# LauraFJulia/TFT_vs_Fund

Measured on AMD Instinct MI355X. Metric: triplet-hypotheses/sec (linearTFT+R,t) at N=200 corresp., higher is better.
Workload: dtype f64; 1 GPU; configs[1]: batch of 10000 synthetic triplets x 200 correspondences, sigma=1px, linearTFT + R_t_from_TFT (LinearTFTPoseEstimation without Reconst), one batch per GPU; batch_per_gpu=10000, correspondences=200, streams=2 (consecutive batches alternate between streams and may overlap), gather=none (1 GPU), failed_triplets=0, warmup_steps_run=2560

## Files before the change

tft_vs_fund_amd/csrc/f_rows_kernel.h:

```cpp
#pragma once
#include "tft_rows_kernel.h"
#include "tft_rows_exact_kernel.h"
#include "f_kernel.h"

namespace tff {

__device__ __forceinline__ void rows_distances_moments_f(const RowSrc& s, const int N, const double (&c)[6], double* nrm, double* nrm2, double* mom) {
    const int p = rows_p();
    double acc[80];
#pragma unroll
    for (int k = 0; k < 80; ++k) acc[k] = 0.0;
    double d[3] = {0.0, 0.0, 0.0};
    Pt6 pnext = rows_load(s, (p < N) ? p : 0);
#pragma unroll 1
    for (int i = p; i < N; i += ROWL) {
        const Pt6 q = pnext;
        if (i + ROWL < N) pnext = rows_load(s, i + ROWL);
        const double x1 = q.v[0] - c[0], y1 = q.v[1] - c[1];
        const double x2 = q.v[2] - c[2], y2 = q.v[3] - c[3];
        const double x3 = q.v[4] - c[4], y3 = q.v[5] - c[5];
        const double m1[6] = {x1 * x1, x1 * y1, x1, y1 * y1, y1, 1.0};
        const double m2[6] = {x2 * x2, x2 * y2, x2, y2 * y2, y2, 1.0};
        const double m3[6] = {x3 * x3, x3 * y3, x3, y3 * y3, y3, 1.0};
        d[0] += sqrt_nonneg(m1[0] + m1[3]); d[1] += sqrt_nonneg(m2[0] + m2[3]); d[2] += sqrt_nonneg(m3[0] + m3[3]);
// ... 67 lines not shown
        const int v2 = p + 1;
        Mat3 F;
#pragma unroll
        for (int r = 0; r < 3; ++r)
#pragma unroll
            for (int c = 0; c < 3; ++c) F.m[r][c] = Fm[9 * p + 3 * r + c];
        F = mat3_mul(mat3_mul(mat3_T(normal_matrix(nrm2, v2)), F), normal_matrix(nrm2, 0));
        double v3[3], fv[3];
        nok = null3<false>(F, v3);
#pragma unroll
        for (int r = 0; r < 3; ++r) fv[r] = F.m[r][0] * v3[0] + F.m[r][1] * v3[1] + F.m[r][2] * v3[2];
#pragma unroll
        for (int r = 0; r < 3; ++r)
#pragma unroll
            for (int c = 0; c < 3; ++c) F.m[r][c] -= fv[r] * v3[c];
        if constexpr (X_FRAME) {
            double nn = 0.0;
#pragma unroll
            for (int r = 0; r < 3; ++r)
#pragma unroll
                for (int c = 0; c < 3; ++c) nn += F.m[r][c] * F.m[r][c];
            const double sc = rsqrt(nn);
#pragma unroll
            for (int r = 0; r < 3; ++r)
#pragma unroll
                for (int c = 0; c < 3; ++c) Fm[9 * p + 3 * r + c] = F.m[r][c] * sc;
        } else {
            F = mat3_mul(mat3_mul(mat3_T(normal_matrix(w->nrm, v2)), F), normal_matrix(w->nrm, 0));
            const Mat3 E = mat3_mul(mat3_mul(mat3_T(load_K(w->calm, v2)), F), load_K(w->calm, 0));
#pragma unroll
            for (int r = 0; r < 3; ++r)
#pragma unroll
                for (int c = 0; c < 3; ++c) rt->Ein[9 * p + 3 * r + c] = E.m[r][c];
        }
    }
    const bool bad = row_any(!nok);
    wave_sync();
    return ok && !bad;
}

template <bool RAGGED>
__device__ __forceinline__ void linear_f_pose_rows(const LinearTftArgs& a) {
    TFF_DYNAMIC_LDS(double, smem);
    if (a.retry_zero && blockIdx.x == 0 && threadIdx.x == 0) *a.retry_zero = 0;
    const int p = lane_id() & 15, row = lane_id() >> 4;
    RowLds* w = reinterpret_cast<RowLds*>(smem) + row;
    RowRt* rt = reinterpret_cast<RowRt*>(w->ov);
    for (long blk = blockIdx.x; RAGGED ? rows_ragged_slot(a, blk) < a.rrange[1] : blk * ROW_TRIPLETS < a.B; blk += gridDim.x) {
        const int N = RAGGED ? rows_ragged_n(a, blk) : opaque_int(a.N);
        const RowJob j = RAGGED ? rows_begin_ragged(a, w, blk) : rows_begin(a, w, blk, N);
        int status;
        if (N < 8) {
            status = ST_TOO_FEW;
            rows_store_nan<RAGGED>(a, j, N);
        } else {
            {
                double cen[6];
                rows_centroids(j.src, N, cen);
                rows_distances_moments_f(j.src, N, cen, w->nrm, w->pa, w->mom);
            }
            wave_sync();
            bool ok = rows_linear_f_middle(w, rt, w->t, w->pa, j.dbg);
            rows_recover_prepare(w, rt);
            status = rows_pose_tail<true, false, RAGGED>(a, w, rt, j, N, ok);
        }
        if (p == 0 && j.valid) {
            if (a.iter) a.iter[j.b] = 0;
            a.status[j.b] = status;
            if (status == ST_RETRY && a.retry_list) a.retry_list[atomicAdd(a.retry_count, 1)] = (int)j.b;
        }
    }
}
__global__ void __launch_bounds__(64, 2) k_linear_f_pose_rows(const LinearTftArgs a) { linear_f_pose_rows<false>(a); }
__global__ void __launch_bounds__(64, 2) k_linear_f_pose_rows_ragged(const LinearTftArgs a) { linear_f_pose_rows<true>(a); }

template <int M>
__device__ __forceinline__ void rows_f_system_chunk(const RowSrc& s, const int N, const int base, const double* nrm, const double* nrm2, const int p, const int ca,
                                                    const int cb, const int pair, double* Rp, double* xch) {
    double a0[M], a1[M];
#pragma unroll
    for (int r = 0; r < M; ++r) {
        const int i = base + r;
        const Pt6 q = premap(premap(rows_load(s, (i < N) ? i : 0), nrm), nrm2);
        const double h1 = (ca == 0) ? q.v[0] : (ca == 1) ? q.v[1] : 1.0;
        const double h2 = (cb == 0) ? (pair ? q.v[4] : q.v[2]) : (cb == 1) ? (pair ? q.v[5] : q.v[3]) : 1.0;
        a0[r] = (i < N && p < 9) ? h1 * h2 : 0.0;
        a1[r] = 0.0;
    }
    rows_qr_append<9, M>(a0, a1, Rp, xch);
}

__device__ __forceinline__ bool rows_linear_f_middle_exact(RowLds* w, RowRt* rt, const RowSrc& s, const int N, double* Fm, double* nrm2, double* dbg) {
    const int p = opaque_lane_int(rows_p());
    double* Rp = w->ov;
    double* xch = w->mom;
    double* dinv = w->mom + 32;
    {
        double sm[6] = {0, 0, 0, 0, 0, 0};
#pragma unroll 1
        for (int i = p; i < N; i += ROWL) {
            const Pt6 q = premap(rows_load(s, i), w->nrm);
#pragma unroll
            for (int k = 0; k < 6; ++k) sm[k] += q.v[k];
        }
        double c[6];
#pragma unroll
        for (int k = 0; k < 6; ++k) c[k] = row_sum16(sm[k]) / (double)N;
        double d[3] = {0.0, 0.0, 0.0};
#pragma unroll 1
        for (int i = p; i < N; i += ROWL) {
            const Pt6 q = premap(rows_load(s, i), w->nrm);
#pragma unroll
            for (int v = 0; v < 3; ++v) {
                const double dx = q.v[2 * v] - c[2 * v], dy = q.v[2 * v + 1] - c[2 * v + 1];
                d[v] += sqrt(dx * dx + dy * dy);
            }
        }
        const double r2c = sqrt(2.0);
#pragma unroll
        for (int v = 0; v < 3; ++v) {
            const double norm0 = row_sum16(d[v]) / (double)N;
            if (p == 3 * v) nrm2[3 * v] = r2c / norm0;
// ... 94 lines not shown
```

tft_vs_fund_amd/csrc/pose_common.h:

```cpp
#pragma once
#include "wave.h"
#include "small_la.h"
#include "wave_eig.h"
#include "row_eig.h"
#include "wave_qr.h"

namespace tff {

constexpr int FLAG_RECONST = 1;
constexpr int FLAG_JACOBI = 2;
constexpr int FLAG_STAGE_LDS = 4;
constexpr int FLAG_ONLY_RETRY = 8;
constexpr int FLAG_DBG_FP_HANDOVER = 64;
constexpr int FLAG_DBG_ADAPTIVE = 32;
constexpr int FLAG_XI_IN_LDS = 128;
constexpr int FLAG_GH_EXACT = 16;

constexpr int ST_OK = 0;
constexpr int ST_TOO_FEW = 1;
constexpr int ST_NONFINITE = 2;
constexpr int ST_NO_POSE = 3;
constexpr int ST_RETRY = 100;

constexpr int DBG_STRIDE = 128;
// ... 419 lines not shown
        double S[4][3];
#pragma unroll
        for (int r = 0; r < 4; ++r)
#pragma unroll
            for (int c = 0; c < 3; ++c) {
                if (c > r) continue;
                double v = b0[r] * b0[c] + b1[r] * b1[c];
                if (r < 3) v += a0[r] * a0[c] + a1[r] * a1[c];
                S[r][c] = v;
            }
        const double S33 = b0[3] * b0[3] + b1[3] * b1[3];
        const double tr3 = S[0][0] + S[1][1] + S[2][2];
        const double delta = 1e-14 * (tr3 + S33), pfloor = 1e-3 * delta + 1e-300;
        double L[4][3], inv[3];
#pragma unroll
        for (int j = 0; j < 3; ++j) {
            double d = S[j][j] + delta;
#pragma unroll
            for (int k = 0; k < j; ++k) d -= L[j][k] * L[j][k];
            d = fmax(d, pfloor);
            inv[j] = rsqrt_pos(d);
#pragma unroll
            for (int r = j + 1; r < 4; ++r) {
                double sv = S[r][j];
#pragma unroll
                for (int k = 0; k < j; ++k) sv -= L[r][k] * L[j][k];
                L[r][j] = sv * inv[j];
            }
        }
        double z[3];
#pragma unroll
        for (int r = 2; r >= 0; --r) {
            double sum = -L[3][r];
#pragma unroll
            for (int k = r + 1; k < 3; ++k) sum -= L[k][r] * z[k];
            z[r] = sum * inv[r];
        }
        const double d1 = z[2], d2 = R3[0] * z[0] + R3[1] * z[1] + R3[2] * z[2] + R3[3];
        const double d4 = S33 + delta - (L[3][0] * L[3][0] + L[3][1] * L[3][1] + L[3][2] * L[3][2]);
        const double zz = z[0] * z[0] + z[1] * z[1] + z[2] * z[2];
        const double idet = (inv[0] * inv[1]) * (inv[0] * inv[1]) * (inv[2] * inv[2]);
        const double trs = tr3 + 3.0 * delta;
        const double e = trs * trs * idet;
        const double Gp = 4.0 * (1.0 + zz) - d4 * e;
        const double rhs = 2.0 * d4 * e + 2.5e-14 * trs * e * Gp;
        const double dmin2 = fmin(d1 * d1, d2 * d2);
        const bool certain = Gp > 0.0 && dmin2 * Gp * Gp > rhs * rhs * zz;
        all_certain = all_certain && certain;
        score += (int)sgn(d1) + (int)sgn(d2);
    }
    return 2 * wave_sum_i(score) + (wave_any(!all_certain) ? 1 : 0);
}
struct VoteCam { double PB[12], R3[4]; };
struct VoteFactor { double L[4][3], inv[3], d4, z[3], pfloor; };
template <bool KEEP = false, bool CERT = true>
__device__ __forceinline__ void vote_one(const double (&SA)[6], const VoteCam& cam, const double x2, const double y2, int& score, bool& all_certain,
                                         VoteFactor* keep = nullptr) {
    double b0[4], b1[4];
#pragma unroll
    for (int c = 0; c < 4; ++c) { b0[c] = y2 * cam.PB[8 + c] - cam.PB[4 + c]; b1[c] = cam.PB[c] - x2 * cam.PB[8 + c]; }
    double S[4][3];
#pragma unroll
    for (int r = 0; r < 4; ++r)
#pragma unroll
        for (int c = 0; c < 3; ++c) {
            if (c > r) continue;
            double v = b0[r] * b0[c] + b1[r] * b1[c];
            if (r < 3) v += SA[r * (r + 1) / 2 + c];
            S[r][c] = v;
        }
    const double S33 = b0[3] * b0[3] + b1[3] * b1[3];
    const double tr3 = S[0][0] + S[1][1] + S[2][2];
    const double delta = 1e-14 * (tr3 + S33), pfloor = 1e-3 * delta + 1e-300;
    double L[4][3], inv[3];
#pragma unroll
    for (int j = 0; j < 3; ++j) {
        double d = S[j][j] + delta;
#pragma unroll
        for (int k = 0; k < j; ++k) d -= L[j][k] * L[j][k];
        d = fmax(d, pfloor);
        inv[j] = rsqrt_pos(d);
#pragma unroll
        for (int r = j + 1; r < 4; ++r) {
            double sv = S[r][j];
#pragma unroll
            for (int k = 0; k < j; ++k) sv -= L[r][k] * L[j][k];
            L[r][j] = sv * inv[j];
        }
    }
    double z[3];
#pragma unroll
    for (int r = 2; r >= 0; --r) {
        double sum = -L[3][r];
#pragma unroll
        for (int k = r + 1; k < 3; ++k) sum -= L[k][r] * z[k];
        z[r] = sum * inv[r];
    }
    const double d4 = S33 + delta - (L[3][0] * L[3][0] + L[3][1] * L[3][1] + L[3][2] * L[3][2]);
    if constexpr (CERT) {
        const double d1 = z[2], d2 = cam.R3[0] * z[0] + cam.R3[1] * z[1] + cam.R3[2] * z[2] + cam.R3[3];
        const double zz = z[0] * z[0] + z[1] * z[1] + z[2] * z[2];
        const double idet = (inv[0] * inv[1]) * (inv[0] * inv[1]) * (inv[2] * inv[2]);
        const double trs = tr3 + 3.0 * delta;
        const double e = trs * trs * idet;
        const double Gp = 4.0 * (1.0 + zz) - d4 * e;
        const double rhs = 2.0 * d4 * e + 2.5e-14 * trs * e * Gp;
        const double dmin2 = fmin(d1 * d1, d2 * d2);
        const bool certain = Gp > 0.0 && dmin2 * Gp * Gp > rhs * rhs * zz;
        all_certain = all_certain && certain;
        score += sgn_i(d1) + sgn_i(d2);
    }
    if constexpr (KEEP) {
#pragma unroll
        for (int r = 0; r < 4; ++r)
#pragma unroll
            for (int c = 0; c < 3; ++c) keep->L[r][c] = (c < r) ? L[r][c] : 0.0;
#pragma unroll
        for (int c = 0; c < 3; ++c) { keep->inv[c] = inv[c]; keep->z[c] = z[c]; }
        keep->d4 = d4;
        keep->pfloor = pfloor;
    }
}
__device__ __forceinline__ bool dlt_from_vote(const VoteFactor& f, double (&X)[4]) {
    double L[4][4], inv[4];
#pragma unroll
    for (int r = 0; r < 4; ++r)
#pragma unroll
        for (int c = 0; c < 4; ++c) L[r][c] = (c < r) ? f.L[r][c] : 0.0;
    inv[0] = f.inv[0]; inv[1] = f.inv[1]; inv[2] = f.inv[2];
    inv[3] = rsqrt_pos(fmax(f.d4, f.pfloor));
    const double nn0 = 1.0 + (f.z[0] * f.z[0] + f.z[1] * f.z[1] + f.z[2] * f.z[2]);
    const double r0 = rsqrt(nn0);
    const bool fin = nn0 <= 1e300;
    X[0] = fin ? f.z[0] * r0 : 0.5; X[1] = fin ? f.z[1] * r0 : 0.5; X[2] = fin ? f.z[2] * r0 : 0.5; X[3] = fin ? r0 : 0.5;
    bool conv;
    chol_invit<4>(L, inv, X, 40, &conv);
    return conv;
}
template <bool CAM1_IN_REGISTERS>
__device__ __attribute__((noinline)) int tri_vote_fast2(PoseLds* w, const double* pts, int N, int view, const double* camB0, const double* Rt0,
                                                        const double* camB1, const double* Rt1) {
    const int lane = lane_id();
    double PA[12];
    VoteCam c0, c1r;
    load_uniform12(w->Pfin[0], PA);
    load_uniform12(camB0, c0.PB);
#pragma unroll
    for (int c = 0; c < 4; ++c) c0.R3[c] = wave_uniform(Rt0[8 + c]);
    if constexpr (CAM1_IN_REGISTERS) {
#pragma unroll
        for (int c = 0; c < 12; ++c) c1r.PB[c] = camB1[c];
#pragma unroll
        for (int c = 0; c < 4; ++c) c1r.R3[c] = Rt1[8 + c];
    }
    int score0 = 0, score1 = 0;
    bool certain0 = true, certain1 = true;
    Pt6 pnext = load_pt(pts, (lane < N) ? lane : 0);
#pragma unroll 1
    for (int i = lane; i < N; i += WAVE) {
        const Pt6 p = pnext;
        if (i + WAVE < N) pnext = load_pt(pts, i + WAVE);
        const double x1 = p.v[0], y1 = p.v[1], x2 = (view == 1) ? p.v[2] : p.v[4], y2 = (view == 1) ? p.v[3] : p.v[5];
        double a0[3], a1[3], SA[6];
#pragma unroll
        for (int c = 0; c < 3; ++c) { a0[c] = y1 * PA[8 + c] - PA[4 + c]; a1[c] = PA[c] - x1 * PA[8 + c]; }
#pragma unroll
        for (int r = 0; r < 3; ++r)
#pragma unroll
            for (int c = 0; c <= r; ++c) SA[r * (r + 1) / 2 + c] = a0[r] * a0[c] + a1[r] * a1[c];
        vote_one(SA, c0, x2, y2, score0, certain0);
        if constexpr (CAM1_IN_REGISTERS) {
            vote_one(SA, c1r, x2, y2, score1, certain1);
        } else {
            VoteCam c1;
            const double* pb = camB1 + opaque_int(0);
            const double* pr = Rt1 + opaque_int(0);
#pragma unroll
            for (int c = 0; c < 12; ++c) c1.PB[c] = pb[c];
#pragma unroll
            for (int c = 0; c < 4; ++c) c1.R3[c] = pr[8 + c];
            vote_one(SA, c1, x2, y2, score1, certain1);
        }
    }
    const int r0 = 2 * wave_sum_i(score0) + (wave_any(!certain0) ? 1 : 0), r1 = 2 * wave_sum_i(score1) + (wave_any(!certain1) ? 1 : 0);
    return (int)(((unsigned)r1 << 16) | ((unsigned)r0 & 0xffffu));
}
__device__ __attribute__((noinline)) int tri_vote_exact(PoseLds* w, const double* pts, int N, int view, const double* camB, const double* Rt) {
// ... 249 lines not shown
```

tft_vs_fund_amd/csrc/tft_rows_kernel.h:

```cpp
#pragma once
#include "tft_kernel.h"
#include "tft_moments_kernel.h"

namespace tff {

constexpr int ROW_TRIPLETS = 4;
constexpr int ROWL = 16;

struct RowRt {
    double T1[28];
    double T2[28];
    double nullv[18];
    double mats[28];
    double Ein[18];
    double cand[2][21];
    double P[4][12];
    double candRt[4][12];
    double Rt[2][12];
    double Pfin[3][12];
};
constexpr int ROW_OV_DOUBLES = 380;
static_assert(sizeof(RowRt) <= ROW_OV_DOUBLES * sizeof(double), "overlay");
struct RowLds {
    double mom[96];
    double nrm[9];
    double calm[27];
    double t[27];
    double epi[6];
    double Q[18];
    double tp[15];
    double pa[18];
    double ov[ROW_OV_DOUBLES];
};
constexpr int ROW_LDS_DOUBLES = (int)(sizeof(RowLds) / sizeof(double));
static_assert(ROW_LDS_DOUBLES % 2 == 0, "16-byte row stride");
inline size_t rows_lds_bytes() { return (size_t)ROW_TRIPLETS * sizeof(RowLds); }
inline unsigned rows_grid(long B) { const long g = (B + ROW_TRIPLETS - 1) / ROW_TRIPLETS; return (unsigned)(g > 0 ? g : 1); }

__device__ __forceinline__ int rows_p() { return lane_id() & 15; }

struct RowSrc { const double* pts; const int* idx; int ns; bool sampled; };
__device__ __forceinline__ Pt6 rows_load(const RowSrc& s, const int i) {
    if (s.sampled) {
        int k = s.idx[i];
        k = (k >= 0 && k < s.ns) ? k : 0;
        return load_pt(s.pts, k);
    }
    return load_pt(s.pts, i);
}

__device__ __forceinline__ void rows_stamp(double* dbg, const int slot) {
    if (dbg) {
        const long long t = shader_clock();
        if (rows_p() == 0) dbg[80 + slot] = (double)t;
    }
}


__device__ __forceinline__ void rows_centroids(const RowSrc& s, const int N, double (&c)[6]) {
    const int p = rows_p();
    double sm[6] = {0, 0, 0, 0, 0, 0};
    int i0 = 0;
#pragma unroll 1
    for (; i0 + 4 * ROWL <= N; i0 += 4 * ROWL) {
        Pt6 q[4];
#pragma unroll
        for (int u = 0; u < 4; ++u) q[u] = rows_load(s, i0 + ROWL * u + p);
#pragma unroll
        for (int u = 0; u < 4; ++u)
#pragma unroll
            for (int k = 0; k < 6; ++k) sm[k] += q[u].v[k];
    }
    if (i0 < N) {
        Pt6 q[4];
#pragma unroll
        for (int u = 0; u < 4; ++u) { const int i = i0 + ROWL * u + p; q[u] = rows_load(s, (i < N) ? i : 0); }
#pragma unroll
        for (int u = 0; u < 4; ++u) {
            const bool have = i0 + ROWL * u + p < N;
#pragma unroll
            for (int k = 0; k < 6; ++k) sm[k] += have ? q[u].v[k] : 0.0;
        }
    }
#pragma unroll
    for (int k = 0; k < 6; ++k) c[k] = row_sum16(sm[k]) / (double)N;
}

__device__ __forceinline__ void rows_distances_moments(const RowSrc& s, const int N, const double (&c)[6], double* nrm, double (&nr)[9], double* mom) {
    const int p = rows_p();
    const int slot = p >> 1;
    const bool odd = (p & 1) != 0;
    double acc[48];
#pragma unroll
    for (int k = 0; k < 48; ++k) acc[k] = 0.0;
    double dA = 0.0, dB = 0.0;
    auto body = [&](const Pt6& q, double& r2_out) {
        const double x1 = q.v[0] - c[0], y1 = q.v[1] - c[1];
        const double x2 = q.v[2] - c[2], y2 = q.v[3] - c[3];
        const double x3 = q.v[4] - c[4], y3 = q.v[5] - c[5];
        const double r1 = x1 * x1 + y1 * y1, r2 = x2 * x2 + y2 * y2, r3 = x3 * x3 + y3 * y3;
        dA += sqrt_nonneg(odd ? r3 : r1);
        r2_out = r2;
        const double q2[4] = {1.0, x2, y2, r2};
        const double q3[4] = {1.0, x3, y3, r3};
        const double pa = odd ? y1 * y1 : x1 * x1, pb = odd ? y1 : x1 * y1, pc = odd ? 1.0 : x1;
#pragma unroll
        for (int b = 0; b < 4; ++b)
#pragma unroll
            for (int cc = 0; cc < 4; ++cc) {
                const double wv = q3[b] * q2[cc];
                acc[4 * b + cc] += pa * wv;
                acc[16 + 4 * b + cc] += pb * wv;
                acc[32 + 4 * b + cc] += pc * wv;
            }
    };
    constexpr int STEP = ROWL / 2;
    Pt6 pe = rows_load(s, (slot < N) ? slot : 0);
    Pt6 po = rows_load(s, (slot + STEP < N) ? slot + STEP : 0);
#pragma unroll 1
    for (int i = slot; i < N; i += 2 * STEP) {
        const Pt6 q = pe;
        if (i + 2 * STEP < N) pe = rows_load(s, i + 2 * STEP);
        double r2a, r2b = 0.0;
        body(q, r2a);
        if (i + STEP < N) {
            const Pt6 r = po;
            if (i + 3 * STEP < N) po = rows_load(s, i + 3 * STEP);
            body(r, r2b);
        }
        dB += sqrt_nonneg(odd ? r2b : r2a);
    }
    const double d1 = row_sum16(odd ? 0.0 : dA), d3 = row_sum16(odd ? dA : 0.0), d2 = row_sum16(dB);
    const double r2c = sqrt(2.0);
    const double dd[3] = {d1, d2, d3};
#pragma unroll
    for (int v = 0; v < 3; ++v) {
        const double norm0 = dd[v] / (double)N;
        nr[3 * v + 0] = r2c / norm0;
        nr[3 * v + 1] = -r2c * c[2 * v] / norm0;
        nr[3 * v + 2] = -r2c * c[2 * v + 1] / norm0;
    }
    if (p < 9) {
        double mine = nr[0];
#pragma unroll
        for (int k = 1; k < 9; ++k) mine = (p == k) ? nr[k] : mine;
        nrm[p] = mine;
    }
#pragma unroll
    for (int i = 0; i < 24; ++i) acc[i] = halve_sum<8>(acc[i], acc[i + 24]);
#pragma unroll
    for (int i = 0; i < 12; ++i) acc[i] = halve_sum<4>(acc[i], acc[i + 12]);
#pragma unroll
    for (int i = 0; i < 6; ++i) acc[i] = halve_sum<2>(acc[i], acc[i + 6]);
    const int base = 6 * ((p >> 1) & 1) + 12 * ((p >> 2) & 1) + 24 * ((p >> 3) & 1);
    const double s1 = nr[0], s2 = nr[3], s3 = nr[6];
#pragma unroll
    for (int i = 0; i < 6; ++i) {
        const int e = 48 * (p & 1) + base + i;
        const int h = e >> 4, i3 = (e >> 2) & 3, i2 = e & 3;
        const double f1 = (h == 5) ? 1.0 : ((h == 2 || h == 4) ? s1 : s1 * s1);
        const double f3 = (i3 == 0) ? 1.0 : ((i3 == 3) ? s3 * s3 : s3);
        const double f2 = (i2 == 0) ? 1.0 : ((i2 == 3) ? s2 * s2 : s2);
        mom[e] = acc[i] * (f1 * f3 * f2);
    }
}

template <int n>
__device__ __forceinline__ void rows_min_eigvec(double (&g0)[RowEigDims<n>::N0], double (&g1)[RowEigDims<n>::N1], const double d0, const double d1,
                                                double* Lp, const int maxit, int* iters, double* resid2, const bool has_start,
                                                const double start0, const double start1, double* gram_risk, double& x0, double& x1,
                                                const double gram_risk_limit2 = 1e14) {
    constexpr int N0 = RowEigDims<n>::N0;
    constexpr bool HI = RowEigDims<n>::HI;
    constexpr int Z = n * (n - 1) / 2;
    const int p = rows_p();
    const bool valid0 = p < n, valid1 = HI && 16 + p < n;
    const double tr = row_sum16((valid0 ? d0 : 0.0) + (valid1 ? d1 : 0.0));
    const double delta = 1e-14 * tr;
    const double pfloor = 1e-3 * delta + 1e-300;
    double myinv0 = 0.0, myinv1 = 0.0;
    RowChol<n, 0>::run(g0, g1, myinv0, myinv1, delta, pfloor, p);
#pragma unroll
    for (int c = 0; c < N0; ++c) g0[c] = (c < p && valid0) ? g0[c] * myinv0 : 0.0;
// ... 282 lines not shown
        const int call = p >> 1, cd = p & 1;
        const Mat3 K = load_K(w->calm, call + 1);
        compose_camera(K, rt->cand[call] + 9 * cd, rt->cand[call] + 18, rt->P[p]);
#pragma unroll
        for (int r = 0; r < 3; ++r) {
#pragma unroll
            for (int c = 0; c < 3; ++c) rt->candRt[p][4 * r + c] = rt->cand[call][9 * cd + 3 * r + c];
            rt->candRt[p][4 * r + 3] = rt->cand[call][18 + r];
        }
    }
    if (p == 4) {
        const Mat3 K1 = load_K(w->calm, 0);
#pragma unroll
        for (int r = 0; r < 3; ++r) { rt->Pfin[0][4 * r] = K1.m[r][0]; rt->Pfin[0][4 * r + 1] = K1.m[r][1]; rt->Pfin[0][4 * r + 2] = K1.m[r][2]; rt->Pfin[0][4 * r + 3] = 0.0; }
    }
    wave_sync();
}

struct RowScale { double num, den; bool conv; bool main1[2]; };
template <bool SPEC = false>
__device__ __forceinline__ bool rows_votes(const RowSrc& s, const int N, const RowRt* rt, const bool all4, int (&sc)[2][2], int* sweeps_out = nullptr,
                                           bool* cert_out = nullptr, RowScale* scale = nullptr) {
    const int p = rows_p();
    double PA[12];
#pragma unroll
    for (int c = 0; c < 12; ++c) PA[c] = rt->Pfin[0][c];
    int scA[2] = {0, 0}, scB[2] = {0, 0};
    bool certA[2] = {true, true}, certB[2] = {true, true};
    int offA[2] = {0, 24}, offB[2] = {12, 36};
    bool main1[2] = {false, false};
    bool evalA = true, evalB[2] = {true, true};
    bool fullB[2] = {true, true};
    bool rowB[2] = {true, true};
    int sweeps = 0;
    double snum = 0.0, sden = 0.0;
    bool sconv = true;
#pragma unroll 1
    for (int sweep = 0; sweep < 2; ++sweep) {
        ++sweeps;
        const int start = (sweep == 0) ? 0 : ROWL;
        Pt6 pnext = rows_load(s, (start + p < N) ? start + p : 0);
#pragma unroll 1
        for (int i0 = start; i0 < N; i0 += ROWL) {
            const Pt6 q = pnext;
            const bool have = i0 + p < N;
            pnext = rows_load(s, (i0 + ROWL + p < N) ? i0 + ROWL + p : 0);
            const double x1 = q.v[0], y1 = q.v[1];
            double a0[3], a1[3], SA[6];
#pragma unroll
            for (int c = 0; c < 3; ++c) { a0[c] = y1 * PA[8 + c] - PA[4 + c]; a1[c] = PA[c] - x1 * PA[8 + c]; }
#pragma unroll
            for (int rr = 0; rr < 3; ++rr)
#pragma unroll
                for (int c = 0; c <= rr; ++c) SA[rr * (rr + 1) / 2 + c] = a0[rr] * a0[c] + a1[rr] * a1[c];
            const bool first = sweep == 0 && i0 == 0;
#pragma unroll
            for (int cc = 0; cc < 2; ++cc) {
                const int call = 1 - cc;
                const double x2 = (call == 0) ? q.v[2] : q.v[4], y2 = (call == 0) ? q.v[3] : q.v[5];
                VoteFactor fA, fB;
                if (evalA) {
                    VoteCam cam;
                    const int off = opaque_lane_int(offA[call]);
                    const double* pb = rt->P[0] + off;
                    const double* pr = rt->candRt[0] + off;
#pragma unroll
                    for (int c = 0; c < 12; ++c) cam.PB[c] = pb[c];
#pragma unroll
                    for (int c = 0; c < 4; ++c) cam.R3[c] = pr[8 + c];
                    int term = 0;
                    bool cert = true;
                    if (SPEC && call == 0 && !first) vote_one<true, false>(SA, cam, x2, y2, term, cert, &fA);
                    else if (SPEC && call == 0) vote_one<true>(SA, cam, x2, y2, term, cert, &fA);
                    else vote_one(SA, cam, x2, y2, term, cert);
                    scA[call] += have ? term : 0;
                    certA[call] = certA[call] && (cert || !have);
                }
                if (evalB[call]) {
                    VoteCam cam;
                    const int off = opaque_lane_int(offB[call]);
                    const double* pb = rt->P[0] + off;
                    const double* pr = rt->candRt[0] + off;
#pragma unroll
                    for (int c = 0; c < 12; ++c) cam.PB[c] = pb[c];
#pragma unroll
                    for (int c = 0; c < 4; ++c) cam.R3[c] = pr[8 + c];
                    int term = 0;
                    bool cert = true;
                    if (SPEC && call == 0 && first) vote_one<true>(SA, cam, x2, y2, term, cert, &fB);
                    else vote_one(SA, cam, x2, y2, term, cert);
                    scB[call] += have ? term : 0;
                    certB[call] = certB[call] && (cert || !have);
                }
                if (first) {
                    const bool v0 = row_any(have && certA[call] && scA[call] != 2), v1 = row_any(have && certA[call] && scA[call] != -2);
                    const bool b0 = row_any(have && certB[call] && scB[call] != 2), b1 = row_any(have && certB[call] && scB[call] != -2);
                    const bool mixA = v0 && v1, mixB = b0 && b1;
                    const bool single = !all4 && (mixA != mixB);
                    main1[call] = single && mixA;
                    if (main1[call]) {
                        const int ts = scA[call]; scA[call] = scB[call]; scB[call] = ts;
                        const bool tc = certA[call]; certA[call] = certB[call]; certB[call] = tc;
                        offA[call] = 12 + 24 * call; offB[call] = 24 * call;
                        if (SPEC && call == 0) fA = fB;
                    }
                    rowB[call] = !single;
                    evalB[call] = wave_any(!single);
                    fullB[call] = evalB[call];
                }
                if (SPEC && call == 0 && evalA) {
                    double X[4];
                    const bool conv = dlt_from_vote(fA, X);
                    sconv = sconv && (conv || !have);
                    if (!first) {
                        const double* pr = rt->candRt[0] + opaque_lane_int(offA[0]);
                        const double s4 = sgn(X[3]);
                        const double d1 = X[2] * s4, d2 = (pr[8] * X[0] + pr[9] * X[1] + pr[10] * X[2] + pr[11] * X[3]) * s4;
                        scA[0] += have ? sgn_i(d1) + sgn_i(d2) : 0;
                        certA[0] = certA[0] && (conv || !have);
                    }
                    const double iw = 1.0 / X[3];
                    const double X0 = X[0] * iw, X1 = X[1] * iw, X2 = X[2] * iw;
                    const double* ax = rt->P[0] + opaque_lane_int(offA[1]);
                    double X3[3], u3[3];
#pragma unroll
                    for (int r = 0; r < 3; ++r) { X3[r] = ax[4 * r] * X0 + ax[4 * r + 1] * X1 + ax[4 * r + 2] * X2; u3[r] = ax[4 * r + 3]; }
                    const double p3[3] = {q.v[4], q.v[5], 1.0};
                    double c1[3], c2[3];
                    cross3(p3, X3, c1);
                    cross3(p3, u3, c2);
                    snum += have ? c1[0] * c2[0] + c1[1] * c2[1] + c1[2] * c2[2] : 0.0;
                    sden += have ? c2[0] * c2[0] + c2[1] * c2[1] + c2[2] * c2[2] : 0.0;
                }
            }
        }
        if (sweep == 1) break;
        bool again = false;
#pragma unroll
        for (int call = 0; call < 2; ++call) {
            const int tA = (int)row_sum16((double)scA[call]);
            const bool mine = !rowB[call] && tA != 2 * N && tA != -2 * N;
            rowB[call] = rowB[call] || mine;
            const bool need = wave_any(!fullB[call] && tA != 2 * N && tA != -2 * N);
            evalB[call] = need;
            fullB[call] = fullB[call] || need;
            again = again || need;
        }
        evalA = false;
        if (!again) break;
    }
    bool ok = true;
#pragma unroll
    for (int call = 0; call < 2; ++call) {
        const int tA = (int)row_sum16((double)scA[call]);
        const int tBsum = (int)row_sum16((double)scB[call]);
        const int tB = (fullB[call] && rowB[call]) ? tBsum : 0;
        const bool badA = row_any(!certA[call]), badB = row_any(!certB[call]);
        ok = ok && !badA && (!(fullB[call] && rowB[call]) || !badB);
        if (cert_out) {
            cert_out[2 * call] = main1[call] ? !badB : !badA;
            cert_out[2 * call + 1] = main1[call] ? !badA : !badB;
        }
        sc[call][0] = main1[call] ? tB : tA;
        sc[call][1] = main1[call] ? tA : tB;
    }
    if constexpr (SPEC) {
        scale->num = row_sum16(snum);
        scale->den = row_sum16(sden);
        scale->conv = !row_any(!sconv);
        scale->main1[0] = main1[0];
        scale->main1[1] = main1[1];
    }
    if (sweeps_out) *sweeps_out = sweeps + (fullB[0] ? 16 : 0) + (fullB[1] ? 32 : 0);
    return ok;
}

// ... 50 lines not shown
    long b;
    bool valid;
    bool bad_index;
    double* dbg;
    RowSrc src;
    long base = 0;
};
__device__ __forceinline__ RowJob rows_begin(const LinearTftArgs& a, RowLds* w, const long blk, const int N) {
    const int lane = lane_id(), p = lane & 15, row = lane >> 4;
    RowJob j;
    const long b_raw = blk * ROW_TRIPLETS + row;
    j.valid = b_raw < a.B;
    j.b = j.valid ? b_raw : a.B - 1;
    j.dbg = a.dbg ? a.dbg + j.b * DBG_STRIDE : nullptr;
    j.src.idx = a.sample_idx ? a.sample_idx + j.b * (long)N : nullptr;
    j.src.pts = a.sample_idx ? a.corresp : a.corresp + j.b * 6 * (long)N;
    j.src.ns = a.sample_ns;
    j.src.sampled = a.sample_idx != nullptr;
    wave_sync();
    j.bad_index = false;
    if (a.sample_idx) {
        bool bad = false;
        for (int i = p; i < N; i += ROWL) { const int k = j.src.idx[i]; bad = bad || !(k >= 0 && k < j.src.ns); }
        j.bad_index = row_any(bad);
    }
    w->calm[p] = a.calm[j.b * a.calm_stride + p];
    if (p < 11) w->calm[16 + p] = a.calm[j.b * a.calm_stride + 16 + p];
    return j;
}
__device__ __forceinline__ long rows_ragged_slot(const LinearTftArgs& a, const long blk) { return a.rrange[0] + blk * ROW_TRIPLETS; }
__device__ __forceinline__ int rows_ragged_n(const LinearTftArgs& a, const long blk) {
    const long b0 = a.rlist[rows_ragged_slot(a, blk)];
    return opaque_int(wave_uniform_i((int)(a.offsets[b0 + 1] - a.offsets[b0])));
}
__device__ __forceinline__ RowJob rows_begin_ragged(const LinearTftArgs& a, RowLds* w, const long blk) {
    const int lane = lane_id(), p = lane & 15, row = lane >> 4;
    const long slot = rows_ragged_slot(a, blk);
    const int e = a.rlist[slot + row];
    RowJob j;
    j.valid = e >= 0;
    j.b = j.valid ? (long)e : (long)a.rlist[slot];
    j.base = a.offsets[j.b];
    j.dbg = nullptr;
    j.src.idx = nullptr;
    j.src.pts = a.corresp + 6 * j.base;
    j.src.ns = 0;
    j.src.sampled = false;
    wave_sync();
    j.bad_index = false;
    w->calm[p] = a.calm[j.b * a.calm_stride + p];
    if (p < 11) w->calm[16 + p] = a.calm[j.b * a.calm_stride + 16 + p];
    return j;
}
template <bool RAGGED = false>
__device__ __forceinline__ void rows_store_nan(const LinearTftArgs& a, const RowJob& j, const int N) {
    const int p = rows_p();
    const double qnan = __longlong_as_double(0x7ff8000000000000LL);
    if (j.valid) {
        if (p < 12) { a.Rt2[j.b * 12 + p] = qnan; a.Rt3[j.b * 12 + p] = qnan; }
        a.T[j.b * 27 + p] = qnan;
        if (p < 11) a.T[j.b * 27 + 16 + p] = qnan;
        if (a.reconst) for (int i = p; i < 3 * N; i += ROWL) a.reconst[(RAGGED ? 3 * j.base : j.b * 3 * (long)N) + i] = qnan;
    }
}

__device__ __forceinline__ int rows_vote_exact(const RowSrc& s, const int N, const RowRt* rt, const int cand_off, const int view) {
    const int p = rows_p();
    typedef const double (&cam_ref)[12];
    cam_ref PA = *reinterpret_cast<const double(*)[12]>(rt->Pfin[0]);
    const double* camB = rt->P[0] + cand_off;
    cam_ref PB = *reinterpret_cast<const double(*)[12]>(camB);
    const double* pr = rt->candRt[0] + cand_off;
    double score = 0.0;
#pragma unroll 1
    for (int i = p; i < N; i += ROWL) {
        const Pt6 q = rows_load(s, i);
        double X[4];
        dlt_point<true, true>(PA, PB, PB, rt->Pfin[0], camB, camB, false, q.v[0], q.v[1], (view == 1) ? q.v[2] : q.v[4], (view == 1) ? q.v[3] : q.v[5], 0.0, 0.0, X);
        const double s4 = sgn(X[3]);
        const double d1 = X[2] * s4, d2 = (pr[8] * X[0] + pr[9] * X[1] + pr[10] * X[2] + pr[11] * X[3]) * s4;
        score += sgn(d1) + sgn(d2);
    }
    return (int)row_sum16(score);
}

__device__ __forceinline__ void rows_vote_exact_pair(const RowSrc& s, const int N, const RowRt* rt, const int k, const int view, int& exA, int& exB) {
    const int p = rows_p(), half = p >> 3, i = p & 7;
    const int cand_off = 12 * (k + half);
    typedef const double (&cam_ref)[12];
    cam_ref PA = *reinterpret_cast<const double(*)[12]>(rt->Pfin[0]);
    const double* camB = rt->P[0] + cand_off;
    cam_ref PB = *reinterpret_cast<const double(*)[12]>(camB);
    const double* pr = rt->candRt[0] + cand_off;
    double score = 0.0;
    if (i < N) {
        const Pt6 q = rows_load(s, i);
        double X[4];
        dlt_point<true, true>(PA, PB, PB, rt->Pfin[0], camB, camB, false, q.v[0], q.v[1], (view == 1) ? q.v[2] : q.v[4], (view == 1) ? q.v[3] : q.v[5], 0.0, 0.0, X);
        const double s4 = sgn(X[3]);
        const double d1 = X[2] * s4, d2 = (pr[8] * X[0] + pr[9] * X[1] + pr[10] * X[2] + pr[11] * X[3]) * s4;
        score = sgn(d1) + sgn(d2);
    }
    exA = (int)row_sum16(half ? 0.0 : score);
    exB = (int)row_sum16(half ? score : 0.0);
}

template <bool T_FROM_CAMERAS, bool EXACT = false, bool RAGGED = false>
__device__ __forceinline__ int rows_pose_tail(const LinearTftArgs& a, RowLds* w, RowRt* rt, const RowJob& j, const int N, bool ok) {
    const int p = rows_p();
    double* dbg = j.dbg;
    const long b = j.b;
    int status = ST_OK;
    RowScale spec;
    spec.num = 0.0; spec.den = 1.0; spec.conv = true; spec.main1[0] = spec.main1[1] = false;
    bool spec_valid = !EXACT;
    double spec_sign = 1.0;
    {
        int sc[2][2];
        int sweeps = 0;
        if constexpr (EXACT) {
            bool cert4[4];
            rows_votes(j.src, N, rt, true, sc, &sweeps, cert4);
            rows_stamp(dbg, 3);
            if (N <= 8) {
#pragma unroll 1
                for (int call = 0; call < 2; ++call) {
                    const bool needA = !(call ? cert4[2] : cert4[0]), needB = !(call ? cert4[3] : cert4[1]);
                    if (!wave_any(needA || needB)) continue;
                    int exA, exB;
                    rows_vote_exact_pair(j.src, N, rt, 2 * call, call + 1, exA, exB);
                    if (needA) { if (call) sc[1][0] = exA; else sc[0][0] = exA; }
                    if (needB) { if (call) sc[1][1] = exB; else sc[0][1] = exB; }
                }
            } else {
#pragma unroll 1
                for (int k = 0; k < 4; ++k) {
                    const bool need = !((k == 0) ? cert4[0] : (k == 1) ? cert4[1] : (k == 2) ? cert4[2] : cert4[3]);
                    if (!wave_any(need)) continue;
                    const int ex = rows_vote_exact(j.src, N, rt, 12 * k, (k < 2) ? 1 : 2);
                    if (need) { if (k == 0) sc[0][0] = ex; else if (k == 1) sc[0][1] = ex; else if (k == 2) sc[1][0] = ex; else sc[1][1] = ex; }
                }
            }
        } else {
            ok = rows_votes<true>(j.src, N, rt, dbg != nullptr && !(a.flags & FLAG_DBG_ADAPTIVE), sc, &sweeps, nullptr, &spec) && ok;
        }
        if (dbg && p == 0) dbg[94] = (double)sweeps;
#pragma unroll
        for (int call = 0; call < 2; ++call) {
            const int sR = sc[call][0], sRp = sc[call][1];
            const int score[4] = {sR, -sR, -sRp, sRp};
            int seen = 0, pick = -1;
#pragma unroll
            for (int k = 0; k < 4; ++k) if (score[k] >= seen) { pick = k; seen = score[k]; }
            if (pick < 0) status = ST_NO_POSE;
            if (dbg && p < 4) dbg[60 + 4 * call + p] = (double)((p == 0) ? score[0] : (p == 1) ? score[1] : (p == 2) ? score[2] : score[3]);
            if (p < 12) {
                const int r = p >> 2, c = p & 3;
                const double* R = rt->cand[call] + ((pick >= 2) ? 9 : 0);
                const double tsign = (pick == 1 || pick == 2) ? -1.0 : 1.0;
                rt->Rt[call][p] = (c < 3) ? R[3 * r + c] : tsign * rt->cand[call][18 + r];
            }
            spec_valid = spec_valid && pick >= 0 && ((pick >= 2) == spec.main1[call]);
            spec_sign = (pick == 1 || pick == 2) ? -spec_sign : spec_sign;
        }
        wave_sync();
    }
    rows_stamp(dbg, 11);
    {
        if (p < 2) compose_camera_from_pose(load_K(w->calm, p + 1), rt->Rt[p], rt->Pfin[p + 1]);
        wave_sync();
        double num = spec_sign * spec.num, den = spec.den;
        bool conv = spec.conv;
        if (dbg && p == 0) dbg[95] = spec_valid ? 1.0 : 0.0;
        if (wave_any(!spec_valid)) {
            double n2, d2;
            const bool c2 = rows_tri_pass<TRI_SCALE, EXACT>(j.src, N, rt->Pfin[0], rt->Pfin[1], rt->Pfin[2], nullptr, n2, d2);
            if (!spec_valid) { num = n2; den = d2; conv = c2; }
        }
        ok = ok && conv;
        const double lam = -num / den;
        if (dbg && p == 0) dbg[68] = lam;
        if (p < 3) rt->Rt[1][4 * p + 3] *= lam;
        wave_sync();
    }
    rows_stamp(dbg, 12);
    if (a.reconst || T_FROM_CAMERAS) {
        if (p == 0) compose_camera_from_pose(load_K(w->calm, 2), rt->Rt[1], rt->Pfin[2]);
        wave_sync();
    }
    if constexpr (T_FROM_CAMERAS) {
        double val[2];
#pragma unroll
        for (int h = 0; h < 2; ++h) {
            const int e = (16 * h + p < 27) ? 16 * h + p : 0;
            const int i = e / 9, k = (e % 9) / 3, jj = e % 3;
            const int r0 = (i == 0) ? 1 : 0, r1 = (i == 2) ? 1 : 2;
            double m[4][4];
#pragma unroll
            for (int c = 0; c < 4; ++c) {
                m[0][c] = rt->Pfin[0][4 * r0 + c];
                m[1][c] = rt->Pfin[0][4 * r1 + c];
                m[2][c] = rt->Pfin[1][4 * jj + c];
                m[3][c] = rt->Pfin[2][4 * k + c];
            }
            val[h] = (16 * h + p < 27) ? ((i == 1) ? -1.0 : 1.0) * det4(m) : 0.0;
        }
        const double rs = rsqrt(row_sum16(val[0] * val[0] + val[1] * val[1]));
        rt->T1[p] = val[0] * rs;
        if (p < 11) rt->T1[16 + p] = val[1] * rs;
        wave_sync();
    }
    double vRt[2], vT[2];
    bool bad = false;
#pragma unroll
    for (int h = 0; h < 2; ++h) {
        const int e24 = 16 * h + p;
        vRt[h] = 0.0; vT[h] = 0.0;
        if (e24 < 24) {
            const int which = e24 / 12, e = e24 % 12, c = e / 3, r = e % 3;
            vRt[h] = rt->Rt[which][4 * r + c];
        }
        if (e24 < 27) vT[h] = rt->T1[e24];
        bad = bad || !(fabs(vRt[h]) <= 1.79e308) || !(fabs(vT[h]) <= 1.79e308);
    }
    const bool nonfinite = row_any(bad);
    if (a.reconst) {
        double n0, d0;
        double* rec = (j.valid && !j.bad_index && !nonfinite) ? a.reconst + (RAGGED ? 3 * j.base : b * 3 * (long)N) : nullptr;
        const bool conv = rows_tri_pass<TRI_RECONST, EXACT>(j.src, N, rt->Pfin[0], rt->Pfin[1], rt->Pfin[2], rec, n0, d0);
        ok = ok && conv;
    }
    if (j.bad_index) status = ST_TOO_FEW;
    else if (!ok) status = ST_RETRY;
    else if (nonfinite && status == ST_OK) status = ST_NONFINITE;
    if (j.bad_index || (ok && nonfinite)) {
        rows_store_nan<RAGGED>(a, j, N);
    } else {
        const bool store = j.valid && ok;
#pragma unroll
        for (int h = 0; h < 2; ++h) {
            const int e24 = 16 * h + p;
            if (e24 < 24 && store) ((e24 >= 12) ? a.Rt3 : a.Rt2)[b * 12 + e24 % 12] = vRt[h];
            if (e24 < 27 && store) a.T[b * 27 + e24] = vT[h];
        }
    }
    rows_stamp(dbg, 13);
    return status;
}

template <bool PRE, bool RAGGED = false>
__global__ void __launch_bounds__(64, 2) k_linear_tft_pose_rows(const LinearTftArgs a) {
    TFF_DYNAMIC_LDS(double, smem);
    if (a.retry_zero && blockIdx.x == 0 && threadIdx.x == 0) *a.retry_zero = 0;
    const int p = lane_id() & 15, row = lane_id() >> 4;
    RowLds* w = reinterpret_cast<RowLds*>(smem) + row;
    RowRt* rt = reinterpret_cast<RowRt*>(w->ov);
    for (long blk = blockIdx.x; RAGGED ? rows_ragged_slot(a, blk) < a.rrange[1] : blk * ROW_TRIPLETS < a.B; blk += gridDim.x) {
        const int N = RAGGED ? rows_ragged_n(a, blk) : opaque_int(a.N);
        const RowJob j = RAGGED ? rows_begin_ragged(a, w, blk) : rows_begin(a, w, blk, N);
        double* dbg = j.dbg;
        rows_stamp(dbg, 0);
        int status;
        if (N < 7) {
            status = ST_TOO_FEW;
            rows_store_nan<RAGGED>(a, j, N);
        } else {
            if constexpr (PRE) {
                rows_load_pre(a.pre, j.b, w->mom, w->nrm);
                rows_stamp(dbg, 1);
                wave_sync();
                if (dbg && p < 9) dbg[71 + p] = w->nrm[p];
            } else {
                double cen[6], nr[9];
                rows_centroids(j.src, N, cen);
                rows_stamp(dbg, 1);
                rows_distances_moments(j.src, N, cen, w->nrm, nr, w->mom);
                if (dbg && p < 9) dbg[71 + p] = w->nrm[p];
            }
            wave_sync();
            rows_stamp(dbg, 2);
            bool ok = rows_linear_tft_middle(w, dbg);
            rows_stamp(dbg, 8);
            rows_transform_tft_inverse(w->t, rt->T1, rt->mats, [w](int v) { return normal_matrix(w->nrm, v); });
            ok = rows_rt_prepare(w, rt, dbg) && ok;
            rows_stamp(dbg, 10);
            status = rows_pose_tail<false, false, RAGGED>(a, w, rt, j, N, ok);
        }
        if (p == 0 && j.valid) {
            if (a.iter) a.iter[j.b] = 0;
            a.status[j.b] = status;
            if (status == ST_RETRY && a.retry_list) a.retry_list[atomicAdd(a.retry_count, 1)] = (int)j.b;
        }
    }
}

}
```

Baseline: 99.50 million triplet-hypotheses/s.

## Reload kernargs late, vectorize LDS camera loads, add FMAs and uniform sqrt

Output pointers and flags are re-read from the kernarg segment just before the stores, so they no longer occupy SGPRs for the whole kernel. Camera matrices in LDS are aligned to 16 bytes and read as paired doubles to cut LDS instruction count. Several multiply-add pairs become explicit fma, the non-finite fallback in dlt_from_vote runs only when some lane needs it, and sqrt in the moments loop uses an rsqrt-based path whose zero check is wave-uniform. These changes aim to lower register pressure and instruction count, at the cost of small last-bit rounding differences.

```diff
diff --git a/tft_vs_fund_amd/csrc/f_rows_kernel.h b/tft_vs_fund_amd/csrc/f_rows_kernel.h
--- a/tft_vs_fund_amd/csrc/f_rows_kernel.h
+++ b/tft_vs_fund_amd/csrc/f_rows_kernel.h
@@ -143,7 +143,7 @@
         int status;
         if (N < 8) {
             status = ST_TOO_FEW;
-            rows_store_nan<RAGGED>(a, j, N);
+            rows_store_nan<RAGGED, true>(a, j, N);
         } else {
             {
                 double cen[6];
@@ -153,12 +153,14 @@
             wave_sync();
             bool ok = rows_linear_f_middle(w, rt, w->t, w->pa, j.dbg);
             rows_recover_prepare(w, rt);
-            status = rows_pose_tail<true, false, RAGGED>(a, w, rt, j, N, ok);
+            status = rows_pose_tail<true, false, RAGGED, true>(a, w, rt, j, N, ok);
         }
         if (p == 0 && j.valid) {
-            if (a.iter) a.iter[j.b] = 0;
-            a.status[j.b] = status;
-            if (status == ST_RETRY && a.retry_list) a.retry_list[atomicAdd(a.retry_count, 1)] = (int)j.b;
+            const auto* al = kernarg_again(a);
+            int* const oiter = al->iter; int* const ostatus = al->status; int* const olist = al->retry_list;
+            if (oiter) oiter[j.b] = 0;
+            ostatus[j.b] = status;
+            if (status == ST_RETRY && olist) olist[atomicAdd(al->retry_count, 1)] = (int)j.b;
         }
     }
 }
diff --git a/tft_vs_fund_amd/csrc/pose_common.h b/tft_vs_fund_amd/csrc/pose_common.h
--- a/tft_vs_fund_amd/csrc/pose_common.h
+++ b/tft_vs_fund_amd/csrc/pose_common.h
@@ -495,6 +495,17 @@
     return 2 * wave_sum_i(score) + (wave_any(!all_certain) ? 1 : 0);
 }
 struct VoteCam { double PB[12], R3[4]; };
+typedef double Pair16 __attribute__((vector_size(16), may_alias));
+template <int K>
+__device__ __forceinline__ void load_pairs16(const double* src, double* dst) {
+    static_assert(K % 2 == 0, "whole pairs");
+    const Pair16* s = reinterpret_cast<const Pair16*>(src);
+#pragma unroll
+    for (int c = 0; c < K; c += 2) {
+        const Pair16 v = s[c / 2];
+        dst[c] = v[0]; dst[c + 1] = v[1];
+    }
+}
 struct VoteFactor { double L[4][3], inv[3], d4, z[3], pfloor; };
 template <bool KEEP = false, bool CERT = true>
 __device__ __forceinline__ void vote_one(const double (&SA)[6], const VoteCam& cam, const double x2, const double y2, int& score, bool& all_certain,
@@ -508,11 +519,11 @@
 #pragma unroll
         for (int c = 0; c < 3; ++c) {
             if (c > r) continue;
-            double v = b0[r] * b0[c] + b1[r] * b1[c];
+            double v = fma(b0[r], b0[c], b1[r] * b1[c]);
             if (r < 3) v += SA[r * (r + 1) / 2 + c];
             S[r][c] = v;
         }
-    const double S33 = b0[3] * b0[3] + b1[3] * b1[3];
+    const double S33 = fma(b0[3], b0[3], b1[3] * b1[3]);
     const double tr3 = S[0][0] + S[1][1] + S[2][2];
     const double delta = 1e-14 * (tr3 + S33), pfloor = 1e-3 * delta + 1e-300;
     double L[4][3], inv[3];
@@ -574,8 +585,12 @@
     inv[3] = rsqrt_pos(fmax(f.d4, f.pfloor));
     const double nn0 = 1.0 + (f.z[0] * f.z[0] + f.z[1] * f.z[1] + f.z[2] * f.z[2]);
     const double r0 = rsqrt(nn0);
-    const bool fin = nn0 <= 1e300;
-    X[0] = fin ? f.z[0] * r0 : 0.5; X[1] = fin ? f.z[1] * r0 : 0.5; X[2] = fin ? f.z[2] * r0 : 0.5; X[3] = fin ? r0 : 0.5;
+    X[0] = f.z[0] * r0; X[1] = f.z[1] * r0; X[2] = f.z[2] * r0; X[3] = r0;
+    if (wave_any(!(nn0 <= 1e300))) {
+        const bool fin = nn0 <= 1e300;
+        X[0] = fin ? X[0] : 0.5; X[1] = fin ? X[1] : 0.5; X[2] = fin ? X[2] : 0.5; X[3] = fin ? X[3] : 0.5;
+        pin_value(X[0]);
+    }
     bool conv;
     chol_invit<4>(L, inv, X, 40, &conv);
     return conv;
diff --git a/tft_vs_fund_amd/csrc/rows_target.h b/tft_vs_fund_amd/csrc/rows_target.h
--- /dev/null
+++ b/tft_vs_fund_amd/csrc/rows_target.h
@@ -0,0 +1,25 @@
+#pragma once
+#include <hip/hip_runtime.h>
+#include <wave_target.h>
+
+namespace tff {
+
+#define TFF_KERNARG_SPACE __attribute__((address_space(4)))
+template <class Args>
+__device__ __forceinline__ const TFF_KERNARG_SPACE Args* kernarg_again(const Args&) {
+    const TFF_KERNARG_SPACE Args* p = (const TFF_KERNARG_SPACE Args*)__builtin_amdgcn_kernarg_segment_ptr();
+    asm volatile("" : "+s"(p));
+    return p;
+}
+
+__device__ __forceinline__ double sqrt_nonneg_uniform(double x) {
+#pragma clang fp contract(off)
+    double s = x * rsqrt_pos(x);
+    if (__ballot(x == 0.0) != 0ull) {
+        s = (x == 0.0) ? 0.0 : s;
+        asm volatile("" : "+v"(s));
+    }
+    return s;
+}
+
+}
diff --git a/tft_vs_fund_amd/csrc/tft_rows_kernel.h b/tft_vs_fund_amd/csrc/tft_rows_kernel.h
--- a/tft_vs_fund_amd/csrc/tft_rows_kernel.h
+++ b/tft_vs_fund_amd/csrc/tft_rows_kernel.h
@@ -1,6 +1,7 @@
 #pragma once
 #include "tft_kernel.h"
 #include "tft_moments_kernel.h"
+#include <rows_target.h>
 
 namespace tff {
 
@@ -14,15 +15,15 @@
     double mats[28];
     double Ein[18];
     double cand[2][21];
-    double P[4][12];
-    double candRt[4][12];
-    double Rt[2][12];
-    double Pfin[3][12];
+    alignas(16) double P[4][12];
+    alignas(16) double candRt[4][12];
+    alignas(16) double Rt[2][12];
+    alignas(16) double Pfin[3][12];
 };
 constexpr int ROW_OV_DOUBLES = 380;
 static_assert(sizeof(RowRt) <= ROW_OV_DOUBLES * sizeof(double), "overlay");
-struct RowLds {
-    double mom[96];
+struct alignas(16) RowLds {
+    alignas(16) double mom[96];
     double nrm[9];
     double calm[27];
     double t[27];
@@ -30,8 +31,10 @@
     double Q[18];
     double tp[15];
     double pa[18];
-    double ov[ROW_OV_DOUBLES];
+    alignas(16) double ov[ROW_OV_DOUBLES];
 };
+static_assert(sizeof(RowLds) == (96 + 9 + 27 + 27 + 6 + 18 + 15 + 18 + ROW_OV_DOUBLES) * sizeof(double), "alignment adds no padding");
+static_assert(sizeof(RowRt) == 318 * sizeof(double) && alignof(RowRt) == 16, "alignment adds no padding");
 constexpr int ROW_LDS_DOUBLES = (int)(sizeof(RowLds) / sizeof(double));
 static_assert(ROW_LDS_DOUBLES % 2 == 0, "16-byte row stride");
 inline size_t rows_lds_bytes() { return (size_t)ROW_TRIPLETS * sizeof(RowLds); }
@@ -99,7 +102,7 @@
         const double x2 = q.v[2] - c[2], y2 = q.v[3] - c[3];
         const double x3 = q.v[4] - c[4], y3 = q.v[5] - c[5];
         const double r1 = x1 * x1 + y1 * y1, r2 = x2 * x2 + y2 * y2, r3 = x3 * x3 + y3 * y3;
-        dA += sqrt_nonneg(odd ? r3 : r1);
+        dA += sqrt_nonneg_uniform(odd ? r3 : r1);
         r2_out = r2;
         const double q2[4] = {1.0, x2, y2, r2};
         const double q3[4] = {1.0, x3, y3, r3};
@@ -128,7 +131,7 @@
             if (i + 3 * STEP < N) po = rows_load(s, i + 3 * STEP);
             body(r, r2b);
         }
-        dB += sqrt_nonneg(odd ? r2b : r2a);
+        dB += sqrt_nonneg_uniform(odd ? r2b : r2a);
     }
     const double d1 = row_sum16(odd ? 0.0 : dA), d3 = row_sum16(odd ? dA : 0.0), d2 = row_sum16(dB);
     const double r2c = sqrt(2.0);
@@ -517,7 +520,7 @@
 #pragma unroll
             for (int rr = 0; rr < 3; ++rr)
 #pragma unroll
-                for (int c = 0; c <= rr; ++c) SA[rr * (rr + 1) / 2 + c] = a0[rr] * a0[c] + a1[rr] * a1[c];
+                for (int c = 0; c <= rr; ++c) SA[rr * (rr + 1) / 2 + c] = fma(a0[rr], a0[c], a1[rr] * a1[c]);
             const bool first = sweep == 0 && i0 == 0;
 #pragma unroll
             for (int cc = 0; cc < 2; ++cc) {
@@ -527,12 +530,8 @@
                 if (evalA) {
                     VoteCam cam;
                     const int off = opaque_lane_int(offA[call]);
-                    const double* pb = rt->P[0] + off;
-                    const double* pr = rt->candRt[0] + off;
-#pragma unroll
-                    for (int c = 0; c < 12; ++c) cam.PB[c] = pb[c];
-#pragma unroll
-                    for (int c = 0; c < 4; ++c) cam.R3[c] = pr[8 + c];
+                    load_pairs16<12>(rt->P[0] + off, cam.PB);
+                    load_pairs16<4>(rt->candRt[0] + off + 8, cam.R3);
                     int term = 0;
                     bool cert = true;
                     if (SPEC && call == 0 && !first) vote_one<true, false>(SA, cam, x2, y2, term, cert, &fA);
@@ -544,12 +543,8 @@
                 if (evalB[call]) {
                     VoteCam cam;
                     const int off = opaque_lane_int(offB[call]);
-                    const double* pb = rt->P[0] + off;
-                    const double* pr = rt->candRt[0] + off;
-#pragma unroll
-                    for (int c = 0; c < 12; ++c) cam.PB[c] = pb[c];
-#pragma unroll
-                    for (int c = 0; c < 4; ++c) cam.R3[c] = pr[8 + c];
+                    load_pairs16<12>(rt->P[0] + off, cam.PB);
+                    load_pairs16<4>(rt->candRt[0] + off + 8, cam.R3);
                     int term = 0;
                     bool cert = true;
                     if (SPEC && call == 0 && first) vote_one<true>(SA, cam, x2, y2, term, cert, &fB);
@@ -578,15 +573,17 @@
                     const bool conv = dlt_from_vote(fA, X);
                     sconv = sconv && (conv || !have);
                     if (!first) {
-                        const double* pr = rt->candRt[0] + opaque_lane_int(offA[0]);
+                        double pr[4];
+                        load_pairs16<4>(rt->candRt[0] + opaque_lane_int(offA[0]) + 8, pr);
                         const double s4 = sgn(X[3]);
-                        const double d1 = X[2] * s4, d2 = (pr[8] * X[0] + pr[9] * X[1] + pr[10] * X[2] + pr[11] * X[3]) * s4;
+                        const double d1 = X[2] * s4, d2 = (pr[0] * X[0] + pr[1] * X[1] + pr[2] * X[2] + pr[3] * X[3]) * s4;
                         scA[0] += have ? sgn_i(d1) + sgn_i(d2) : 0;
                         certA[0] = certA[0] && (conv || !have);
                     }
                     const double iw = 1.0 / X[3];
                     const double X0 = X[0] * iw, X1 = X[1] * iw, X2 = X[2] * iw;
-                    const double* ax = rt->P[0] + opaque_lane_int(offA[1]);
+                    double ax[12];
+                    load_pairs16<12>(rt->P[0] + opaque_lane_int(offA[1]), ax);
                     double X3[3], u3[3];
 #pragma unroll
                     for (int r = 0; r < 3; ++r) { X3[r] = ax[4 * r] * X0 + ax[4 * r + 1] * X1 + ax[4 * r + 2] * X2; u3[r] = ax[4 * r + 3]; }
@@ -743,15 +740,22 @@
     if (p < 11) w->calm[16 + p] = a.calm[j.b * a.calm_stride + 16 + p];
     return j;
 }
-template <bool RAGGED = false>
+template <bool KERNARG>
+__device__ __forceinline__ auto rows_args_at(const LinearTftArgs& a) {
+    if constexpr (KERNARG) return kernarg_again(a);
+    else return &a;
+}
+template <bool RAGGED = false, bool KERNARG = false>
 __device__ __forceinline__ void rows_store_nan(const LinearTftArgs& a, const RowJob& j, const int N) {
     const int p = rows_p();
     const double qnan = __longlong_as_double(0x7ff8000000000000LL);
     if (j.valid) {
-        if (p < 12) { a.Rt2[j.b * 12 + p] = qnan; a.Rt3[j.b * 12 + p] = qnan; }
-        a.T[j.b * 27 + p] = qnan;
-        if (p < 11) a.T[j.b * 27 + 16 + p] = qnan;
-        if (a.reconst) for (int i = p; i < 3 * N; i += ROWL) a.reconst[(RAGGED ? 3 * j.base : j.b * 3 * (long)N) + i] = qnan;
+        const auto* al = rows_args_at<KERNARG>(a);
+        double* const oRt2 = al->Rt2; double* const oRt3 = al->Rt3; double* const oT = al->T; double* const orec = al->reconst;
+        if (p < 12) { oRt2[j.b * 12 + p] = qnan; oRt3[j.b * 12 + p] = qnan; }
+        oT[j.b * 27 + p] = qnan;
+        if (p < 11) oT[j.b * 27 + 16 + p] = qnan;
+        if (orec) for (int i = p; i < 3 * N; i += ROWL) orec[(RAGGED ? 3 * j.base : j.b * 3 * (long)N) + i] = qnan;
     }
 }
 
@@ -796,7 +800,7 @@
     exB = (int)row_sum16(half ? score : 0.0);
 }
 
-template <bool T_FROM_CAMERAS, bool EXACT = false, bool RAGGED = false>
+template <bool T_FROM_CAMERAS, bool EXACT = false, bool RAGGED = false, bool KERNARG = false>
 __device__ __forceinline__ int rows_pose_tail(const LinearTftArgs& a, RowLds* w, RowRt* rt, const RowJob& j, const int N, bool ok) {
     const int p = rows_p();
     double* dbg = j.dbg;
@@ -875,7 +879,8 @@
         wave_sync();
     }
     rows_stamp(dbg, 12);
-    if (a.reconst || T_FROM_CAMERAS) {
+    double* const oreconst = rows_args_at<KERNARG>(a)->reconst;
+    if (oreconst || T_FROM_CAMERAS) {
         if (p == 0) compose_camera_from_pose(load_K(w->calm, 2), rt->Rt[1], rt->Pfin[2]);
         wave_sync();
     }
@@ -915,9 +920,9 @@
         bad = bad || !(fabs(vRt[h]) <= 1.79e308) || !(fabs(vT[h]) <= 1.79e308);
     }
     const bool nonfinite = row_any(bad);
-    if (a.reconst) {
+    if (oreconst) {
         double n0, d0;
-        double* rec = (j.valid && !j.bad_index && !nonfinite) ? a.reconst + (RAGGED ? 3 * j.base : b * 3 * (long)N) : nullptr;
+        double* rec = (j.valid && !j.bad_index && !nonfinite) ? oreconst + (RAGGED ? 3 * j.base : b * 3 * (long)N) : nullptr;
         const bool conv = rows_tri_pass<TRI_RECONST, EXACT>(j.src, N, rt->Pfin[0], rt->Pfin[1], rt->Pfin[2], rec, n0, d0);
         ok = ok && conv;
     }
@@ -925,15 +930,19 @@
     else if (!ok) status = ST_RETRY;
     else if (nonfinite && status == ST_OK) status = ST_NONFINITE;
     if (j.bad_index || (ok && nonfinite)) {
-        rows_store_nan<RAGGED>(a, j, N);
+        rows_store_nan<RAGGED, KERNARG>(a, j, N);
     } else {
         const bool store = j.valid && ok;
-#pragma unroll
-        for (int h = 0; h < 2; ++h) {
-            const int e24 = 16 * h + p;
-            if (e24 < 24 && store) ((e24 >= 12) ? a.Rt3 : a.Rt2)[b * 12 + e24 % 12] = vRt[h];
-            if (e24 < 27 && store) a.T[b * 27 + e24] = vT[h];
-        }
+        auto stores = [&](const auto* al) {
+            double* const oRt2 = al->Rt2; double* const oRt3 = al->Rt3; double* const oT = al->T;
+#pragma unroll
+            for (int h = 0; h < 2; ++h) {
+                const int e24 = 16 * h + p;
+                if (e24 < 24 && store) ((e24 >= 12) ? oRt3 : oRt2)[b * 12 + e24 % 12] = vRt[h];
+                if (e24 < 27 && store) oT[b * 27 + e24] = vT[h];
+            }
+        };
+        stores(rows_args_at<KERNARG>(a));
     }
     rows_stamp(dbg, 13);
     return status;
@@ -954,7 +963,7 @@
         int status;
         if (N < 7) {
             status = ST_TOO_FEW;
-            rows_store_nan<RAGGED>(a, j, N);
+            rows_store_nan<RAGGED, true>(a, j, N);
         } else {
             if constexpr (PRE) {
                 rows_load_pre(a.pre, j.b, w->mom, w->nrm);
@@ -975,14 +984,16 @@
             rows_transform_tft_inverse(w->t, rt->T1, rt->mats, [w](int v) { return normal_matrix(w->nrm, v); });
             ok = rows_rt_prepare(w, rt, dbg) && ok;
             rows_stamp(dbg, 10);
-            status = rows_pose_tail<false, false, RAGGED>(a, w, rt, j, N, ok);
+            status = rows_pose_tail<false, false, RAGGED, true>(a, w, rt, j, N, ok);
         }
         if (p == 0 && j.valid) {
-            if (a.iter) a.iter[j.b] = 0;
-            a.status[j.b] = status;
-            if (status == ST_RETRY && a.retry_list) a.retry_list[atomicAdd(a.retry_count, 1)] = (int)j.b;
-        }
-    }
-}
-
-}
+            const auto* al = kernarg_again(a);
+            int* const oiter = al->iter; int* const ostatus = al->status; int* const olist = al->retry_list;
+            if (oiter) oiter[j.b] = 0;
+            ostatus[j.b] = status;
+            if (status == ST_RETRY && olist) olist[atomicAdd(al->retry_count, 1)] = (int)j.b;
+        }
+    }
+}
+
+}
```

Result: faster. 102.9 million triplet-hypotheses/s (median of 6 runs) (+3.4%).
